# zeux/phyx

Measured on AMD Instinct MI355X. Metric: solver joint-visits/s (contacts/sec) on the 200k-box stack scene; solver iterations/s in extra, higher is better.
Workload: dtype f32

## Files before the change

phyx_amd/csrc/broadphase.hip:

```cpp
#include "handles.h"
#include "device_scan.h"
#include "device_radix.h"
#include "splitter_sort.h"

#include <algorithm>

namespace phx {

static inline int grid_for(int n, int per_block = 256, int cap = 4096) { return std::max(1, std::min(div_up(n, per_block), cap)); }

__device__ __forceinline__ unsigned radix_float(float v)
{
    const int f = __float_as_int(v);
    const unsigned mask = (unsigned)(f >> 31) | 0x80000000u;
    return (unsigned)f ^ mask;
}

__global__ void __launch_bounds__(256) k_extract_aabb(const phx_rigid_body* __restrict__ bodies, int n, float4* __restrict__ aabb)
{
    for (int i = blockIdx.x * blockDim.x + threadIdx.x; i < n; i += gridDim.x * blockDim.x)
        aabb[i] = make_float4(bodies[i].aabb_min.x, bodies[i].aabb_min.y, bodies[i].aabb_max.x, bodies[i].aabb_max.y);
}

template <bool INTEGRATE>
__global__ void __launch_bounds__(256) k_build_keys(const float4* __restrict__ aabb, float4* __restrict__ vel, const float4* __restrict__ mpos, int n,
                                                    unsigned* __restrict__ keys, unsigned* __restrict__ idx,
                                                    unsigned long long* __restrict__ small, int nsmall, unsigned* __restrict__ chunk_count, int nchunks,
                                                    unsigned long long* __restrict__ stamps, float gravity, float dt, unsigned* __restrict__ counters, const float4* __restrict__ accel)
{
    if (INTEGRATE && blockIdx.x == 0 && threadIdx.x < 8) counters[threadIdx.x] = 0u;
    if (blockIdx.x == 0 && threadIdx.x == 0) { stamps[0] = (unsigned long long)wall_clock64(); stamps[1] = 0ull; }
    for (int i = blockIdx.x * blockDim.x + threadIdx.x; i < nsmall; i += gridDim.x * blockDim.x) small[i] = 0ull;
    for (int i = blockIdx.x * blockDim.x + threadIdx.x; i < nchunks; i += gridDim.x * blockDim.x) chunk_count[i] = 0u;
    for (int i = blockIdx.x * blockDim.x + threadIdx.x; i < n; i += gridDim.x * blockDim.x) {
        keys[i] = radix_float(aabb[i].x);
        idx[i] = (unsigned)i;
        if (INTEGRATE) {
            float4 v = vel[i];
            float ax = 0.f, ay = 0.f, aa = 0.f;
            if (accel) { const float4 a = accel[i]; ax = a.x; ay = a.y; aa = a.z; }
            if (mpos[i].x > 0.0f) ay += gravity;
            v.x += ax * dt; v.y += ay * dt;
            v.z += aa * dt;
            vel[i] = v;
        }
    }
}

__global__ void __launch_bounds__(256) k_gather_entries(const float4* __restrict__ aabb, const unsigned* __restrict__ keys, const unsigned* __restrict__ idx, int n,
                                                        float4* __restrict__ entries, unsigned long long* __restrict__ splitters, int stride)
{
    for (int i = blockIdx.x * blockDim.x + threadIdx.x; i < n; i += gridDim.x * blockDim.x) {
        const float4 b = aabb[idx[i]];
        const float minx = b.x, miny = b.y, maxx = b.z, maxy = b.w;
        entries[i] = make_float4(minx, maxx, (miny + maxy) * 0.5f, (maxy - miny) * 0.5f);
        if (i && i % stride == 0) splitters[i / stride - 1] = ((unsigned long long)keys[i] << 32) | idx[i];
    }
}

constexpr unsigned long long PS_EMPTY = 0xFFFFFFFFFFFFFFFFull;
constexpr unsigned long long PS_TOMB = 0xFFFFFFFFFFFFFFFEull;

__device__ __forceinline__ unsigned ps_hash(unsigned long long k)
{
    const unsigned lb = (unsigned)(k >> 32), rb = (unsigned)k;
    return (lb ^ (rb + 0x9e3779b9u + (lb << 6) + (lb >> 2))) * 0x9E3779B1u;
}

__device__ __forceinline__ bool ps_contains(const unsigned long long* __restrict__ table, unsigned mask, unsigned long long k)
{
    unsigned p = ps_hash(k) & mask;
    for (;;) {
        const unsigned long long s = table[p];
        if (s == k) return true;
        if (s == PS_EMPTY) return false;
        p = (p + 1) & mask;
    }
}

__global__ void __launch_bounds__(256) k_ps_insert(unsigned long long* table, unsigned mask, const uint2* __restrict__ pairs, int n, unsigned long long* __restrict__ end_stamp)
{
    for (int i = blockIdx.x * blockDim.x + threadIdx.x; i < n; i += gridDim.x * blockDim.x) {
        const unsigned long long k = ((unsigned long long)pairs[i].x << 32) | pairs[i].y;
        unsigned p = ps_hash(k) & mask;
        for (;;) {
            const unsigned long long s = table[p];
            if (s == PS_EMPTY || s == PS_TOMB) {
                if (atomicCAS(&table[p], s, k) == s) break;
                continue;
            }
            p = (p + 1) & mask;
        }
    }
    if (end_stamp && threadIdx.x == 0) atomicMax(end_stamp, (unsigned long long)wall_clock64());
}

__global__ void __launch_bounds__(256) k_ps_erase(unsigned long long* table, unsigned mask, const uint2* __restrict__ pairs, int n, int* erased)
{
    int mine = 0;
    for (int i = blockIdx.x * blockDim.x + threadIdx.x; i < n; i += gridDim.x * blockDim.x) {
        const unsigned long long k = ((unsigned long long)pairs[i].x << 32) | pairs[i].y;
        unsigned p = ps_hash(k) & mask;
        for (;;) {
            const unsigned long long s = table[p];
            if (s == k) { table[p] = PS_TOMB; ++mine; break; }
            if (s == PS_EMPTY) break;
            p = (p + 1) & mask;
        }
    }
    for (int off = 32; off > 0; off >>= 1) mine += __shfl_down(mine, off);
    if ((threadIdx.x & 63) == 0 && mine) atomicAdd(erased, mine);
}

__global__ void __launch_bounds__(256) k_ps_rehash(const unsigned long long* __restrict__ old_table, unsigned old_cap,
                                                   unsigned long long* table, unsigned mask)
{
    for (unsigned i = blockIdx.x * blockDim.x + threadIdx.x; i < old_cap; i += gridDim.x * blockDim.x) {
        const unsigned long long k = old_table[i];
        if (k == PS_EMPTY || k == PS_TOMB) continue;
        unsigned p = ps_hash(k) & mask;
        for (;;) {
            if (table[p] == PS_EMPTY && atomicCAS(&table[p], PS_EMPTY, k) == PS_EMPTY) break;
            p = (p + 1) & mask;
        }
    }
}

constexpr int STAT_SLOTS = 64;
constexpr int ROW_CACHE = 4;
constexpr int HUB_LEN = 2048;
constexpr int HUB_CHUNK = 512;

struct SweepView {
    const float4* entries;
    const unsigned* idx;
    int n;
    const unsigned long long* table;
    unsigned mask;
    unsigned* row_count;
    unsigned* row_cache;
    int* cache_overflow;
    int4* chunks;
    unsigned* chunk_count;
    int* n_chunks;
    int chunk_cap;
    unsigned long long* counters;
};

struct FilteredSweepView : SweepView {
    const uint4* filters;
};
template <class V> struct SweepFilter { static constexpr bool on = false; };
template <> struct SweepFilter<FilteredSweepView> { static constexpr bool on = true; };
template <class V> __device__ __forceinline__ uint4 sweep_filter_of(const V& v, unsigned body)
{
    if constexpr (SweepFilter<V>::on) return v.filters[body];
    else return make_uint4(0u, 0u, 0u, 0u);
}

constexpr int SWEEP_CAND = 16;
constexpr int SWEEP_LOOK = 8;
constexpr int SWEEP_GROUP = 8;

__device__ __forceinline__ int scan_end(const float4* __restrict__ entries, int n, int i, float maxx)
{
    int lo = i + 1, hi = n;
    while (lo < hi) {
        const int mid = (lo + hi) >> 1;
        if (entries[mid].x > maxx) hi = mid; else lo = mid + 1;
    }
    return lo;
}

#define PHX_SWEEP_WAVE_SYNC() do { __builtin_amdgcn_fence(__ATOMIC_RELEASE, "wavefront"); __builtin_amdgcn_wave_barrier(); __builtin_amdgcn_fence(__ATOMIC_ACQUIRE, "wavefront"); } while (0)

template <bool EMIT, class V>
__global__ void __launch_bounds__(256) k_sweep_rows(V v, const unsigned* __restrict__ row_offset, uint2* __restrict__ out, unsigned total)
{
    __shared__ unsigned cand[SWEEP_CAND][256];
    __shared__ float4 stage[4][2][64];
    unsigned long long tests = 0, overlaps = 0;
    const int lane = threadIdx.x & 63;
    for (int base = blockIdx.x * blockDim.x + (threadIdx.x & ~63); base < v.n; base += gridDim.x * blockDim.x) {
        const int i = base + lane;
        const bool in_range = i < v.n;
        const float4 a = in_range ? v.entries[i] : make_float4(0.f, 0.f, 0.f, 0.f);
        const bool hub = in_range && i + 1 + HUB_LEN < v.n && !(v.entries[i + 1 + HUB_LEN].x > a.y);
        if (!EMIT) {
            int end = 0, nc = 0, first = 0;
            if (hub) {
                end = scan_end(v.entries, v.n, i, a.y);
                const int len = end - i - 1;
                nc = (len + HUB_CHUNK - 1) / HUB_CHUNK;
                first = atomicAdd(v.n_chunks, nc);
                v.row_count[i] = 0;
                tests += (unsigned long long)len;
            }
            for (unsigned long long hubs = __ballot(hub); hubs; hubs &= hubs - 1ull) {
                const int l = __builtin_ctzll(hubs);
                const int hi = __shfl(i, l), hend = __shfl(end, l), hnc = __shfl(nc, l), hfirst = __shfl(first, l);
                for (int k = lane; k < hnc && hfirst + k < v.chunk_cap; k += 64)
                    v.chunks[hfirst + k] = make_int4(hi, hi + 1 + k * HUB_CHUNK, min(hend, hi + 1 + (k + 1) * HUB_CHUNK), hfirst);
            }
        }
        bool scanning = in_range && !hub;
        const unsigned dst = EMIT && scanning ? row_offset[i] : 0u;
        if (EMIT && scanning) {
            const unsigned next = i + 1 < v.n ? row_offset[i + 1] : total;
            if (next - dst <= (unsigned)ROW_CACHE) scanning = false;
        }
        const unsigned ia = scanning ? v.idx[i] : 0u;
        const uint4 fa = scanning ? sweep_filter_of(v, ia) : make_uint4(0u, 0u, 0u, 0u);
        unsigned found = 0;
        int ncand = 0;
        auto flush = [&]() {
            for (int h = 0; h < ncand; h += SWEEP_LOOK) {
                unsigned ib[SWEEP_LOOK];
                unsigned long long first[SWEEP_LOOK];
#pragma unroll
                for (int k = 0; k < SWEEP_LOOK; ++k) ib[k] = h + k < ncand ? v.idx[cand[h + k][threadIdx.x]] : 0u;
                unsigned pass = ~0u;
                if constexpr (SweepFilter<V>::on) {
                    pass = 0u;
#pragma unroll
                    for (int k = 0; k < SWEEP_LOOK; ++k)
                        if (h + k < ncand && collision_filter_pass(fa, sweep_filter_of(v, ib[k]))) pass |= 1u << k;
                }
#pragma unroll
                for (int k = 0; k < SWEEP_LOOK; ++k) first[k] = h + k < ncand && ((pass >> k) & 1u) ? v.table[ps_hash(((unsigned long long)ia << 32) | ib[k]) & v.mask] : 0ull;
#pragma unroll
                for (int k = 0; k < SWEEP_LOOK; ++k) {
                    if (h + k >= ncand) break;
                    if (!((pass >> k) & 1u)) continue;
                    const unsigned long long key = ((unsigned long long)ia << 32) | ib[k];
                    bool present = first[k] == key;
                    if (!present && first[k] != PS_EMPTY) present = ps_contains(v.table, v.mask, key);
                    if (!present) {
                        if (EMIT) out[dst + found] = make_uint2(ia, ib[k]);
                        else if (found < (unsigned)ROW_CACHE) v.row_cache[(size_t)i * ROW_CACHE + found] = ib[k];
                        ++found;
                    }
                }
            }
            ncand = 0;
        };
        int len = 0;
        bool ended = !scanning;
        int ended_w = scanning ? 0 : -1;
        const int c0 = __builtin_amdgcn_readfirstlane(base) + 1;
        float4* my_stage = &stage[threadIdx.x >> 6][0][0];
        float4 nxt = v.entries[min(c0 + lane, v.n - 1)];
        int buf = 0;
        for (int c = c0; c < v.n && __ballot(!ended); c += 64) {
            my_stage[buf * 64 + lane] = nxt;
            if (c + 64 < v.n) nxt = v.entries[min(c + 64 + lane, v.n - 1)];
            PHX_SWEEP_WAVE_SYNC();
            const float4* blockp = my_stage + buf * 64;
            const int rel = i - c;
            for (int g = 0; g < 64 && c + g < v.n && __ballot(!ended); g += SWEEP_GROUP) {
                if (ncand > SWEEP_CAND - SWEEP_GROUP) flush();
                float4 b[SWEEP_GROUP];
#pragma unroll
                for (int k = 0; k < SWEEP_GROUP; ++k) b[k] = blockp[g + k];
#pragma unroll
                for (int k = 0; k < SWEEP_GROUP; ++k) {
                    const int j = c + g + k;
                    const int started = (rel - (g + k)) >> 31;
                    const int in_list = (j - v.n) >> 31;
                    const int beyond = b[k].x > a.y ? -1 : 0;
                    const int live = started & in_list & ~ended_w;
                    ended_w |= live & beyond;
                    const int tested = live & ~beyond;
                    len -= tested;
                    const int ov = (fabsf(b[k].z - a.z) <= a.w + b[k].w ? -1 : 0) & tested;
                    if (__any(ov)) {
                        if (ov) {
                            if (!EMIT) ++overlaps;
                            cand[ncand++][threadIdx.x] = (unsigned)j;
                        }
                    }
                }
                ended = ended_w != 0;
            }
            buf ^= 1;
        }
        if (scanning) {
            flush();
            if (!EMIT) { v.row_count[i] = found; tests += (unsigned long long)len; if (found > (unsigned)ROW_CACHE) *v.cache_overflow = 1; }
        }
    }
    if (!EMIT) {
        for (int off = 32; off > 0; off >>= 1) { tests += __shfl_down(tests, off); overlaps += __shfl_down(overlaps, off); }
        __shared__ unsigned long long part[2][4];
        if ((threadIdx.x & 63) == 0) { part[0][threadIdx.x >> 6] = tests; part[1][threadIdx.x >> 6] = overlaps; }
        __syncthreads();
        if (threadIdx.x < 2) {
            const unsigned long long t = part[threadIdx.x][0] + part[threadIdx.x][1] + part[threadIdx.x][2] + part[threadIdx.x][3];
            if (t) atomicAdd(&v.counters[2 * (blockIdx.x % STAT_SLOTS) + threadIdx.x], t);
        }
    }
}
__device__ __forceinline__ void emit_cached_rows(const SweepView& v, const unsigned* __restrict__ row_offset, uint2* __restrict__ out, unsigned total, int block, int blocks)
{
    for (int i = block * (int)blockDim.x + (int)threadIdx.x; i < v.n; i += blocks * (int)blockDim.x) {
        const unsigned dst = row_offset[i];
        const unsigned count = (i + 1 < v.n ? row_offset[i + 1] : total) - dst;
        if (count == 0 || count > (unsigned)ROW_CACHE) continue;
        if (i + 1 + HUB_LEN < v.n && !(v.entries[i + 1 + HUB_LEN].x > v.entries[i].y)) continue;
        const unsigned ia = v.idx[i];
        for (unsigned k = 0; k < count; ++k) out[dst + k] = make_uint2(ia, v.row_cache[(size_t)i * ROW_CACHE + k]);
    }
}

template <bool EMIT, class V>
__device__ __forceinline__ void sweep_chunks(const V& v, const unsigned* __restrict__ row_offset, uint2* __restrict__ out, int block, int blocks)
{
    __shared__ unsigned wave_cnt[4];
    __shared__ unsigned running;
    const int total = min(*v.n_chunks, v.chunk_cap);
    const int wave = threadIdx.x >> 6, lane = threadIdx.x & 63;
    unsigned long long overlaps_all = 0;
    for (int c = block; c < total; c += blocks) {
        const int4 ch = v.chunks[c];
        const float4 a = v.entries[ch.x];
        const unsigned ia = v.idx[ch.x];
        const uint4 fa = sweep_filter_of(v, ia);
        unsigned long long overlaps = 0;
        if constexpr (!EMIT) {
            unsigned mine = 0;
            for (int j = ch.y + (int)threadIdx.x; j < ch.z; j += 256) {
                const float4 b = v.entries[j];
                if (fabsf(b.z - a.z) <= a.w + b.w) {
                    ++overlaps;
                    const unsigned ib = v.idx[j];
                    if (SweepFilter<V>::on && !collision_filter_pass(fa, sweep_filter_of(v, ib))) continue;
                    if (!ps_contains(v.table, v.mask, ((unsigned long long)ia << 32) | ib)) ++mine;
                }
            }
            for (int off = 32; off > 0; off >>= 1) mine += __shfl_down(mine, off);
            if (lane == 0) wave_cnt[wave] = mine;
            __syncthreads();
            if (threadIdx.x == 0) v.chunk_count[c] = wave_cnt[0] + wave_cnt[1] + wave_cnt[2] + wave_cnt[3];
            overlaps_all += overlaps;
            __syncthreads();
            continue;
        }
        if (threadIdx.x == 0) running = row_offset[ch.x] + v.chunk_count[c];
        __syncthreads();
        for (int j0 = ch.y; j0 < ch.z; j0 += 256) {
            const int j = j0 + threadIdx.x;
            bool hit = false;
            unsigned ib = 0;
            if (j < ch.z) {
                const float4 b = v.entries[j];
                if (fabsf(b.z - a.z) <= a.w + b.w) {
                    ib = v.idx[j];
                    ++overlaps;
                    hit = (!SweepFilter<V>::on || collision_filter_pass(fa, sweep_filter_of(v, ib))) && !ps_contains(v.table, v.mask, ((unsigned long long)ia << 32) | ib);
                }
            }
            const unsigned long long bal = __ballot(hit);
            if (lane == 0) wave_cnt[wave] = (unsigned)__popcll(bal);
            __syncthreads();
            unsigned before = 0;
            for (int w = 0; w < wave; ++w) before += wave_cnt[w];
            const unsigned base = running;
            if (EMIT && hit) out[base + before + (unsigned)__popcll(bal & ((1ull << lane) - 1ull))] = make_uint2(ia, ib);
            __syncthreads();
            if (threadIdx.x == 0) running = base + wave_cnt[0] + wave_cnt[1] + wave_cnt[2] + wave_cnt[3];
            __syncthreads();
        }
        __syncthreads();
    }
    if (!EMIT) {
        for (int off = 32; off > 0; off >>= 1) overlaps_all += __shfl_down(overlaps_all, off);
        if (lane == 0 && overlaps_all) atomicAdd(&v.counters[2 * ((block * 4 + wave) % STAT_SLOTS) + 1], overlaps_all);
    }
}

template <class V>
__global__ void __launch_bounds__(256) k_sweep_chunks_count(V v) { sweep_chunks<false>(v, nullptr, nullptr, (int)blockIdx.x, (int)gridDim.x); }

template <class V>
__global__ void __launch_bounds__(256) k_emit_pairs(V v, const unsigned* __restrict__ row_offset, uint2* __restrict__ out, unsigned total, int row_blocks)
{
    if ((int)blockIdx.x < row_blocks) emit_cached_rows(v, row_offset, out, total, (int)blockIdx.x, row_blocks);
    else sweep_chunks<true>(v, row_offset, out, (int)blockIdx.x - row_blocks, (int)gridDim.x - row_blocks);
}

__global__ void __launch_bounds__(1024) k_chunk_bases(SweepView v, unsigned* __restrict__ scanned)
{
    __shared__ unsigned lds[16];
    __shared__ unsigned tot;
    const int total = min(*v.n_chunks, v.chunk_cap);
    unsigned carry = 0;
    for (int tile = 0; tile < total; tile += 1024) {
        const int c = tile + (int)threadIdx.x;
        const unsigned mine = c < total ? v.chunk_count[c] : 0u;
        const unsigned ex = block_exclusive_scan_1024(mine, lds, threadIdx.x == 0 ? &tot : nullptr);
        if (c < total) scanned[c] = carry + ex;
        __syncthreads();
        carry += tot;
        __syncthreads();
    }
    __threadfence_block();
    __syncthreads();
    for (int c = threadIdx.x; c < total; c += 1024) {
        const int4 ch = v.chunks[c];
        const unsigned count = v.chunk_count[c];
        const bool last = (c + 1 == total) || v.chunks[c + 1].x != ch.x;
        if (last) v.row_count[ch.x] = scanned[c] + count - scanned[ch.w];
    }
    __syncthreads();
    for (int c = threadIdx.x; c < total; c += 1024) v.chunk_count[c] = scanned[c] - scanned[v.chunks[c].w];
}

__global__ void __launch_bounds__(256) k_entries_to_aos(const float4* __restrict__ entries, const unsigned* __restrict__ keys,
                                                        const unsigned* __restrict__ idx, int n,
                                                        phx_broadphase_entry* __restrict__ out_entries, phx_sort_entry* __restrict__ out_sorted)
{
    for (int i = blockIdx.x * blockDim.x + threadIdx.x; i < n; i += gridDim.x * blockDim.x) {
        const float4 e = entries[i];
        out_entries[i].minx = e.x; out_entries[i].maxx = e.y; out_entries[i].centery = e.z; out_entries[i].extenty = e.w;
        out_entries[i].index = idx[i];
        out_sorted[i].value = keys[i]; out_sorted[i].index = idx[i];
    }
}


DeviceBroadphase::~DeviceBroadphase()
{
    if (hipSetDevice(device_) != hipSuccess) return;
    if (stream_) (void)hipStreamSynchronize(stream_);
    if (stream_) (void)hipStreamDestroy(stream_);
}

int DeviceBroadphase::init()
{
    PHX_TRY(use_device(device_));
    PHX_HIP(hipStreamCreateWithFlags(&stream_, hipStreamNonBlocking));
    PHX_TRY(small_.reserve(16 + 2 * STAT_SLOTS));
    PHX_TRY(erase_count_.reserve(1));
    PHX_HIP(hipMemsetAsync(erase_count_.p, 0, sizeof(int), stream_));
    return clear();
}

int DeviceBroadphase::exclusive_scan(unsigned* data, int count, unsigned* total_out)
{
    return device_exclusive_scan(data, count, total_out, scan_tiles_, stream_);
}

int DeviceBroadphase::resize_table(unsigned want_cap)
{
    unsigned cap = 1024;
    while (cap < want_cap) cap <<= 1;
    DevBuf<unsigned long long> fresh;
    PHX_TRY(fresh.reserve(cap));
    PHX_HIP(hipMemsetAsync(fresh.p, 0xFF, (size_t)cap * sizeof(unsigned long long), stream_));
    if (table_.p && table_cap_) {
        hipLaunchKernelGGL(k_ps_rehash, dim3(grid_for((int)table_cap_)), dim3(256), 0, stream_, table_.p, table_cap_, fresh.p, cap - 1);
        PHX_HIP(hipGetLastError());
    }
    PHX_HIP(hipStreamSynchronize(stream_));
    table_ = std::move(fresh);
    table_cap_ = cap;
    tombstones_ = 0;
    return PHX_OK;
}

int DeviceBroadphase::clear()
{
    PHX_TRY(use_device(device_));
    table_.release();
    table_cap_ = 0;
    set_size_ = 0;
    tombstones_ = 0;
    if (erase_unchecked_) { erase_unchecked_ = 0; PHX_HIP(hipMemsetAsync(erase_count_.p, 0, sizeof(int), stream_)); }
    return resize_table(1024);
}

int DeviceBroadphase::update_device(const phx_rigid_body* d_bodies, int n)
{
    PHX_TRY(use_device(device_));
    PHX_REQUIRE(n >= 0 && (n == 0 || d_bodies), "bad body array");
    PHX_TRY(st_aabb_.reserve(std::max(n, 1)));
    if (n) hipLaunchKernelGGL(k_extract_aabb, dim3(grid_for(n)), dim3(256), 0, stream_, d_bodies, n, st_aabb_.p);
    PHX_HIP(hipGetLastError());
    return update_resident(st_aabb_.p, n);
}

int DeviceBroadphase::update_resident(const float4* d_bodies, int n, const StepPrologue* prologue, const std::function<int()>* while_waiting, const MailCarrier* carrier,
                                      const uint4* filters)
{
    PHX_TRY(use_device(device_));
    PHX_REQUIRE(n >= 0 && (n == 0 || d_bodies), "bad body array");
    n_ = n;
    last_new_ = 0;
    stats_ = phx_broadphase_stats{};
    for (int k = 0; k < 2; ++k) { PHX_TRY(keys_[k].reserve(std::max(n, 1))); PHX_TRY(idx_[k].reserve(std::max(n, 1))); }
    PHX_TRY(hist_.reserve(radix_hist_words(n)));
    int chunk_cap = std::max<int>((int)chunks_.cap, div_up(std::max(n, 1), HUB_CHUNK) * 8 + 64);
    PHX_TRY(chunks_.reserve(chunk_cap));
    PHX_TRY(chunk_count_.reserve(chunk_cap));
    PHX_TRY(entries_.reserve(std::max(n, 1)));
    PHX_TRY(row_count_.reserve(std::max(n, 1) + 1));
    PHX_TRY(row_cache_.reserve((size_t)std::max(n, 1) * ROW_CACHE));
    if ((unsigned long long)(set_size_ + tombstones_) * 2 > table_cap_) PHX_TRY(resize_table((unsigned)std::max<long long>(4 * set_size_, 1024)));

    PHX_TRY(stamps_.reserve(2));
    if (n == 0) {
        if (prologue) PHX_HIP(hipMemsetAsync(prologue->counters, 0, 8 * sizeof(unsigned), stream_));
        PHX_HIP(hipMemsetAsync(stamps_.p, 0, 2 * sizeof(unsigned long long), stream_));
        PHX_HIP(hipStreamSynchronize(stream_));
        stats_.candidate_tests = 0; stats_.overlapping_pairs = 0; stats_.new_pairs = 0; last_new_ = 0;
        stats_.set_size = (int)set_size_; have_update_ = true; ms_pending_ = true;
        return PHX_OK;
    }

    const int buckets = ss_buckets(n);
    const bool appended = splitters_n_ == n && splitters_from_ > 0 && splitters_from_ < n;
    const int deal = appended ? ss_buckets(splitters_from_) : buckets;
    PHX_TRY(splitters_.reserve(SS_MAX_BUCKETS)); PHX_TRY(ss_stats_.reserve(2));
    static const bool no_split = getenv("PHX_NO_SPLIT_SORT") != nullptr;
    const bool split = !no_split && buckets <= SS_MAX_BUCKETS && (buckets == 1 || (splitters_n_ == n && !split_unbalanced_ && (!appended || n <= 2 * splitters_from_)));
    int src = 0;
    if (split) {
        if (!ss_count_.p) { PHX_TRY(ss_count_.reserve(2 * SS_MAX_BUCKETS)); PHX_HIP(hipMemsetAsync(ss_count_.p, 0, ss_count_.cap * sizeof(unsigned), stream_)); }
        PHX_TRY(ss_base_.reserve(SS_MAX_BUCKETS + 1)); PHX_TRY(bucket_of_.reserve(n)); PHX_TRY(bucketed_.reserve(n));
        SplitSortView sv{};
        sv.aabb = d_bodies; sv.n = n; sv.buckets = deal; sv.stride = ss_stride(n); sv.splitters = splitters_.p; sv.keys = keys_[0].p; sv.bucket_of = bucket_of_.p;
        sv.count = ss_count_.p; sv.cursor = ss_count_.p + SS_MAX_BUCKETS; sv.base = ss_base_.p; sv.bucketed = bucketed_.p;
        sv.keys_out = keys_[1].p; sv.idx_out = idx_[1].p; sv.entries = entries_.p; sv.next_splitters = splitters_.p; sv.max_bucket = ss_stats_.p;
        const int items = ss_tile_items(deal);
        const dim3 tiles(div_up(n, SS_TILE_T * items));
#define PHX_KEYS_BUCKETS(INTEGRATE, ITEMS, ...) hipLaunchKernelGGL((k_keys_buckets<INTEGRATE, ITEMS>), tiles, dim3(SS_TILE_T), 0, stream_, sv, __VA_ARGS__)
        if (prologue) {
            if (items == SS_ITEMS_LARGE) PHX_KEYS_BUCKETS(true, SS_ITEMS_LARGE, prologue->vel, prologue->mpos, small_.p, 16 + 2 * STAT_SLOTS, chunk_count_.p, chunk_cap, stamps_.p, prologue->gravity, prologue->dt, prologue->counters, prologue->accel);
            else PHX_KEYS_BUCKETS(true, SS_ITEMS_SMALL, prologue->vel, prologue->mpos, small_.p, 16 + 2 * STAT_SLOTS, chunk_count_.p, chunk_cap, stamps_.p, prologue->gravity, prologue->dt, prologue->counters, prologue->accel);
        } else {
            if (items == SS_ITEMS_LARGE) PHX_KEYS_BUCKETS(false, SS_ITEMS_LARGE, (float4*)nullptr, (const float4*)nullptr, small_.p, 16 + 2 * STAT_SLOTS, chunk_count_.p, chunk_cap, stamps_.p, 0.f, 0.f, (unsigned*)nullptr, (const float4*)nullptr);
            else PHX_KEYS_BUCKETS(false, SS_ITEMS_SMALL, (float4*)nullptr, (const float4*)nullptr, small_.p, 16 + 2 * STAT_SLOTS, chunk_count_.p, chunk_cap, stamps_.p, 0.f, 0.f, (unsigned*)nullptr, (const float4*)nullptr);
        }
#undef PHX_KEYS_BUCKETS
        if (items == SS_ITEMS_LARGE) hipLaunchKernelGGL((k_bucket_scatter<SS_ITEMS_LARGE>), tiles, dim3(SS_TILE_T), 0, stream_, sv);
        else hipLaunchKernelGGL((k_bucket_scatter<SS_ITEMS_SMALL>), tiles, dim3(SS_TILE_T), 0, stream_, sv);
        if (ss_last_max_ <= (unsigned)SS_LDS_SMALL_LIMIT) hipLaunchKernelGGL((k_bucket_sort<SS_LDS_SMALL>), dim3(deal), dim3(SS_SORT_T), 0, stream_, sv);
        else hipLaunchKernelGGL((k_bucket_sort<SS_LDS_RECORDS>), dim3(deal), dim3(SS_SORT_T), 0, stream_, sv);
        src = 1;
    } else {
        if (prologue) hipLaunchKernelGGL((k_build_keys<true>), dim3(grid_for(n)), dim3(256), 0, stream_, d_bodies, prologue->vel, prologue->mpos, n, keys_[0].p, idx_[0].p, small_.p, 16 + 2 * STAT_SLOTS,
                                         chunk_count_.p, chunk_cap, stamps_.p, prologue->gravity, prologue->dt, prologue->counters, prologue->accel);
        else hipLaunchKernelGGL((k_build_keys<false>), dim3(grid_for(n)), dim3(256), 0, stream_, d_bodies, (float4*)nullptr, (const float4*)nullptr, n, keys_[0].p, idx_[0].p, small_.p, 16 + 2 * STAT_SLOTS,
                                chunk_count_.p, chunk_cap, stamps_.p, 0.f, 0.f, (unsigned*)nullptr, (const float4*)nullptr);
        PHX_TRY(device_radix_sort_pairs(keys_[0].p, idx_[0].p, keys_[1].p, idx_[1].p, n, 32, hist_.p, scan_tiles_, stream_, &src));
        hipLaunchKernelGGL(k_gather_entries, dim3(grid_for(n)), dim3(256), 0, stream_, d_bodies, (const unsigned*)keys_[src].p, (const unsigned*)idx_[src].p, n, entries_.p, splitters_.p, ss_stride(n));
        PHX_HIP(hipMemsetAsync(ss_stats_.p, 0, sizeof(unsigned), stream_));
        split_unbalanced_ = false;
    }
    sorted_ = src;
    splitters_n_ = n; splitters_from_ = n;
    split_sorted_ = split;

    SweepView v{};
    v.entries = entries_.p; v.idx = idx_[src].p; v.n = n; v.table = table_.p; v.mask = table_cap_ - 1;
    v.row_count = row_count_.p; v.row_cache = row_cache_.p; v.cache_overflow = reinterpret_cast<int*>(small_.p + 4);
    v.n_chunks = reinterpret_cast<int*>(small_.p + 2);
    v.counters = small_.p + 16;
    unsigned long long host_small[16 + 2 * STAT_SLOTS] = {0};
    int chunk_grid = 1;
    for (int attempt = 0;; ++attempt) {
        v.chunks = chunks_.p; v.chunk_count = chunk_count_.p; v.chunk_cap = chunk_cap;
        chunk_grid = std::min(chunk_cap, 2048);
        if (filters) {
            const FilteredSweepView fv{v, filters};
            hipLaunchKernelGGL((k_sweep_rows<false, FilteredSweepView>), dim3(grid_for(n)), dim3(256), 0, stream_, fv, (const unsigned*)nullptr, (uint2*)nullptr, 0u);
            hipLaunchKernelGGL((k_sweep_chunks_count<FilteredSweepView>), dim3(chunk_grid), dim3(256), 0, stream_, fv);
        } else {
            hipLaunchKernelGGL((k_sweep_rows<false, SweepView>), dim3(grid_for(n)), dim3(256), 0, stream_, v, (const unsigned*)nullptr, (uint2*)nullptr, 0u);
            hipLaunchKernelGGL((k_sweep_chunks_count<SweepView>), dim3(chunk_grid), dim3(256), 0, stream_, v);
        }
        PHX_TRY(chunk_scan_.reserve(chunk_cap + 1));
        hipLaunchKernelGGL(k_chunk_bases, dim3(1), dim3(1024), 0, stream_, v, chunk_scan_.p);
        PHX_TRY(exclusive_scan(row_count_.p, n, reinterpret_cast<unsigned*>(small_.p + 3)));
        PHX_HIP(hipGetLastError());
        int erased = 0;
        PHX_TRY(queue_erase_check(&erased));
        PHX_TRY(rb_.add(host_small, small_.p, sizeof host_small, stream_));
        unsigned max_bucket = 0;
        if (split) PHX_TRY(rb_.add(&max_bucket, ss_stats_.p, sizeof max_bucket, stream_));
        PHX_TRY(rb_.wait(stream_, stamps_.p + 1, attempt == 0 ? while_waiting : nullptr, attempt == 0 ? carrier : nullptr));
        PHX_TRY(settle_erase_check(erased));
        ss_last_max_ = split ? max_bucket : 0u;
        if (split && max_bucket > (unsigned)(4 * ss_stride(n))) split_unbalanced_ = true;
        const int needed = (int)(host_small[2] & 0xFFFFFFFFull);
        if (needed <= chunk_cap) break;
        if (attempt) { set_error("broadphase: hub chunk list overflow twice (%d chunks)", needed); return PHX_ERR_CAPACITY; }
        chunk_cap = needed + 64;
        PHX_TRY(chunks_.reserve(chunk_cap));
        PHX_TRY(chunk_count_.reserve(chunk_cap));
        PHX_HIP(hipMemsetAsync(small_.p, 0, (16 + 2 * STAT_SLOTS) * sizeof(unsigned long long), stream_));
        PHX_HIP(hipMemsetAsync(chunk_count_.p, 0, (size_t)chunk_cap * sizeof(unsigned), stream_));
    }
    const unsigned total = (unsigned)host_small[3];
    stats_.candidate_tests = 0; stats_.overlapping_pairs = 0;
    for (int k = 0; k < STAT_SLOTS; ++k) { stats_.candidate_tests += (long long)host_small[16 + 2 * k]; stats_.overlapping_pairs += (long long)host_small[17 + 2 * k]; }
    stats_.new_pairs = (int)total;
    last_new_ = (int)total;
    if (total) {
        PHX_TRY(new_pairs_.reserve(total));
        if ((unsigned long long)(set_size_ + tombstones_ + (long long)total) * 2 > table_cap_)
            PHX_TRY(resize_table((unsigned)std::min<long long>(4ll * (set_size_ + (long long)total), 1ll << 30)));
        v.table = table_.p; v.mask = table_cap_ - 1;
        {
            const int row_blocks = grid_for(n), chunk_blocks = (host_small[2] & 0xFFFFFFFFull) ? std::min((int)(host_small[2] & 0xFFFFFFFFull), chunk_grid) : 0;
            if (filters) hipLaunchKernelGGL((k_emit_pairs<FilteredSweepView>), dim3(row_blocks + chunk_blocks), dim3(256), 0, stream_, FilteredSweepView{v, filters}, (const unsigned*)row_count_.p, new_pairs_.p, total, row_blocks);
            else hipLaunchKernelGGL((k_emit_pairs<SweepView>), dim3(row_blocks + chunk_blocks), dim3(256), 0, stream_, v, (const unsigned*)row_count_.p, new_pairs_.p, total, row_blocks);
        }
        if (host_small[4] & 0xFFFFFFFFull) {
            if (filters) hipLaunchKernelGGL((k_sweep_rows<true, FilteredSweepView>), dim3(grid_for(n)), dim3(256), 0, stream_, FilteredSweepView{v, filters}, (const unsigned*)row_count_.p, new_pairs_.p, total);
            else hipLaunchKernelGGL((k_sweep_rows<true, SweepView>), dim3(grid_for(n)), dim3(256), 0, stream_, v, (const unsigned*)row_count_.p, new_pairs_.p, total);
        }
        hipLaunchKernelGGL(k_ps_insert, dim3(grid_for((int)total)), dim3(256), 0, stream_, table_.p, table_cap_ - 1, (const uint2*)new_pairs_.p, (int)total, stamps_.p + 1);
        PHX_HIP(hipGetLastError());
        set_size_ += total;
    }
    stats_.set_size = (int)set_size_;
    have_update_ = true;
    ms_pending_ = true;
    return PHX_OK;
}

int DeviceBroadphase::update_host(const phx_rigid_body* bodies, int n, uint32_t* new_pairs, int cap, int* count)
{
    PHX_TRY(use_device(device_));
    PHX_REQUIRE(n >= 0 && (n == 0 || bodies), "bad body array");
    PHX_TRY(st_bodies_.reserve(std::max(n, 1)));
    if (n) PHX_HIP(hipMemcpyAsync(st_bodies_.p, bodies, (size_t)n * sizeof(phx_rigid_body), hipMemcpyHostToDevice, stream_));
    PHX_TRY(update_device(st_bodies_.p, n));
    PHX_HIP(hipStreamSynchronize(stream_));
    return get_new_pairs(new_pairs, cap, count);
}

int DeviceBroadphase::get_new_pairs(uint32_t* out, int cap, int* count)
{
    if (!have_update_) { set_error("no broadphase update has run yet"); return PHX_ERR_STATE; }
    if (count) *count = last_new_;
    if (!out) return PHX_OK;
    if (cap < last_new_) { set_error("new-pair buffer too small: need %d", last_new_); return PHX_ERR_CAPACITY; }
    PHX_TRY(use_device(device_));
    PHX_HIP(hipStreamSynchronize(stream_));
    if (last_new_) PHX_HIP(hipMemcpy(out, new_pairs_.p, (size_t)last_new_ * sizeof(uint2), hipMemcpyDeviceToHost));
    return PHX_OK;
}

int DeviceBroadphase::get_sorted(phx_sort_entry* sorted, phx_broadphase_entry* entries, int cap)
{
    if (!have_update_) { set_error("no broadphase update has run yet"); return PHX_ERR_STATE; }
    if (cap < n_) { set_error("sorted buffers too small: need %d", n_); return PHX_ERR_CAPACITY; }
    PHX_TRY(use_device(device_));
    if (!n_) return PHX_OK;
    DevBuf<phx_broadphase_entry> de;
    DevBuf<phx_sort_entry> ds;
    PHX_TRY(de.reserve(n_));
    PHX_TRY(ds.reserve(n_));
    hipLaunchKernelGGL(k_entries_to_aos, dim3(grid_for(n_)), dim3(256), 0, stream_, (const float4*)entries_.p, (const unsigned*)keys_[sorted_].p,
                       (const unsigned*)idx_[sorted_].p, n_, de.p, ds.p);
    PHX_HIP(hipGetLastError());
    if (entries) PHX_HIP(hipMemcpyAsync(entries, de.p, (size_t)n_ * sizeof(phx_broadphase_entry), hipMemcpyDeviceToHost, stream_));
    if (sorted) PHX_HIP(hipMemcpyAsync(sorted, ds.p, (size_t)n_ * sizeof(phx_sort_entry), hipMemcpyDeviceToHost, stream_));
    PHX_HIP(hipStreamSynchronize(stream_));
    de.release();
    ds.release();
    return PHX_OK;
}

int DeviceBroadphase::erase_pairs_device(const uint2* d_pairs, int count)
{
    PHX_TRY(use_device(device_));
    PHX_REQUIRE(count >= 0 && (count == 0 || d_pairs), "bad pair list");
    if (!count) return PHX_OK;
    hipLaunchKernelGGL(k_ps_erase, dim3(grid_for(count)), dim3(256), 0, stream_, table_.p, table_cap_ - 1, d_pairs, count, erase_count_.p);
    PHX_HIP(hipGetLastError());
    set_size_ -= count;
    tombstones_ += count;
    erase_unchecked_ += count;
    return PHX_OK;
}

int DeviceBroadphase::reset_pairs(const uint2* pairs, int count)
{
    PHX_TRY(use_device(device_));
    PHX_REQUIRE(count >= 0 && (count == 0 || pairs), "bad pair list");
    if (count) {
        PHX_TRY(scratch_pairs_.reserve((size_t)count));
        PHX_HIP(hipMemcpyAsync(scratch_pairs_.p, pairs, (size_t)count * sizeof(uint2), hipMemcpyHostToDevice, stream_));
    }
    PHX_TRY(reset_pairs_device(scratch_pairs_.p, count));
    PHX_HIP(hipStreamSynchronize(stream_));
    return PHX_OK;
}

int DeviceBroadphase::reset_pairs_device(const uint2* d_pairs, int count)
{
    PHX_TRY(use_device(device_));
    PHX_REQUIRE(count >= 0 && (count == 0 || d_pairs), "bad pair list");
    PHX_TRY(clear());
    have_update_ = false;
    if (!count) return PHX_OK;
    PHX_TRY(resize_table(4u * (unsigned)count + 1024u));
    hipLaunchKernelGGL(k_ps_insert, dim3(grid_for(count)), dim3(256), 0, stream_, table_.p, table_cap_ - 1, d_pairs, count, (unsigned long long*)nullptr);
    PHX_HIP(hipGetLastError());
    set_size_ = count;
    stats_.set_size = count;
    return PHX_OK;
}

int DeviceBroadphase::queue_erase_check(int* erased)
{
    *erased = 0;
    if (!erase_unchecked_) return PHX_OK;
    return rb_.add(erased, erase_count_.p, sizeof(int), stream_);
}

int DeviceBroadphase::settle_erase_check(int erased)
{
    if (!erase_unchecked_) return PHX_OK;
    const long long missing = erase_unchecked_ - erased;
    set_size_ += missing;
    tombstones_ = std::max<long long>(0, tombstones_ - missing);
    erase_unchecked_ = 0;
    PHX_HIP(hipMemsetAsync(erase_count_.p, 0, sizeof(int), stream_));
    return PHX_OK;
}

int DeviceBroadphase::erase_pairs(const uint32_t* pairs, int count)
{
    PHX_TRY(use_device(device_));
    PHX_REQUIRE(count >= 0 && (count == 0 || pairs), "bad pair list");
    if (!count) return PHX_OK;
    PHX_TRY(scratch_pairs_.reserve(count));
    PHX_HIP(hipMemcpyAsync(scratch_pairs_.p, pairs, (size_t)count * sizeof(uint2), hipMemcpyHostToDevice, stream_));
    return erase_pairs_device(scratch_pairs_.p, count);
}

int DeviceBroadphase::get_stats(phx_broadphase_stats* out)
{
    PHX_REQUIRE(out, "null out");
    if (!have_update_) { set_error("no broadphase update has run yet"); return PHX_ERR_STATE; }
    PHX_TRY(use_device(device_));
    if (ms_pending_) {
        unsigned long long stamps[2] = {0, 0};
        PHX_TRY(rb_.add(stamps, stamps_.p, sizeof stamps, stream_));
        PHX_TRY(rb_.wait(stream_));
        stats_.device_ms = stamps[1] > stamps[0] ? (double)(stamps[1] - stamps[0]) * 1e-5 : 0.0;
        ms_pending_ = false;
    }
    if (erase_unchecked_) {
        int erased = 0;
        PHX_TRY(queue_erase_check(&erased));
        PHX_TRY(rb_.wait(stream_));
        PHX_TRY(settle_erase_check(erased));
    }
    *out = stats_;
    out->set_size = (int)set_size_;
    return PHX_OK;
}

}


extern "C" {

int phx_broadphase_create(phx_broadphase** out, int device)
{
    PHX_REQUIRE(out, "null out");
    *out = nullptr;
    PHX_TRY(phx::use_device(device));
    phx_broadphase* b = new (std::nothrow) phx_broadphase(device);
    PHX_REQUIRE(b, "out of host memory");
    int st = b->impl.init();
    if (st != PHX_OK) { delete b; return st; }
    *out = b;
    return PHX_OK;
}

void phx_broadphase_destroy(phx_broadphase* b) { delete b; }

int phx_broadphase_clear(phx_broadphase* b) { PHX_REQUIRE(b, "null handle"); return b->impl.clear(); }

int phx_broadphase_update(phx_broadphase* b, const phx_rigid_body* bodies, int32_t n, uint32_t* new_pairs, int32_t cap, int32_t* count)
{
    PHX_REQUIRE(b, "null handle");
    return b->impl.update_host(bodies, n, new_pairs, cap, count);
}

int phx_broadphase_update_device(phx_broadphase* b, const void* d_bodies, int32_t n)
{
    PHX_REQUIRE(b, "null handle");
    return b->impl.update_device(static_cast<const phx_rigid_body*>(d_bodies), n);
}

int phx_broadphase_get_sorted(phx_broadphase* b, phx_sort_entry* sorted, phx_broadphase_entry* entries, int32_t cap)
{
    PHX_REQUIRE(b, "null handle");
    return b->impl.get_sorted(sorted, entries, cap);
}

int phx_broadphase_get_new_pairs(phx_broadphase* b, uint32_t* new_pairs, int32_t cap, int32_t* count)
{
    PHX_REQUIRE(b, "null handle");
    return b->impl.get_new_pairs(new_pairs, cap, count);
}

int phx_broadphase_erase_pairs(phx_broadphase* b, const uint32_t* pairs, int32_t count)
{
    PHX_REQUIRE(b, "null handle");
    return b->impl.erase_pairs(pairs, count);
}

int phx_broadphase_get_stats(phx_broadphase* b, phx_broadphase_stats* out)
{
    PHX_REQUIRE(b, "null handle");
    return b->impl.get_stats(out);
}

}
```

Before: 116.8 billion.

## Fuse pair-set insertion into broadphase emit kernels and drop separate insert pass

New pairs are now inserted into the persistent pair hash table right where they are written out (emit_cached_rows, sweep_chunks, and the emit variant of k_sweep_rows), and the separate k_ps_insert launch after emission is removed. The end timestamp moves into whichever emit kernel runs last, and only a subset of blocks issue the atomicMax. This saves one kernel launch and a re-read of the new-pairs buffer. The risk is that emit kernels probing the table with ps_contains now race with concurrent inserts into the same table, and the insert loop was changed to reuse the CAS return value.

Result: no change. 116.9 billion (median of 3 runs) (+0.1%).

```diff
diff --git a/phyx_amd/csrc/broadphase.hip b/phyx_amd/csrc/broadphase.hip
--- a/phyx_amd/csrc/broadphase.hip
+++ b/phyx_amd/csrc/broadphase.hip
@@ -78,21 +78,31 @@
     }
 }
 
-__global__ void __launch_bounds__(256) k_ps_insert(unsigned long long* table, unsigned mask, const uint2* __restrict__ pairs, int n, unsigned long long* __restrict__ end_stamp)
-{
-    for (int i = blockIdx.x * blockDim.x + threadIdx.x; i < n; i += gridDim.x * blockDim.x) {
-        const unsigned long long k = ((unsigned long long)pairs[i].x << 32) | pairs[i].y;
-        unsigned p = ps_hash(k) & mask;
-        for (;;) {
-            const unsigned long long s = table[p];
-            if (s == PS_EMPTY || s == PS_TOMB) {
-                if (atomicCAS(&table[p], s, k) == s) break;
-                continue;
-            }
-            p = (p + 1) & mask;
-        }
-    }
-    if (end_stamp && threadIdx.x == 0) atomicMax(end_stamp, (unsigned long long)wall_clock64());
+__device__ __forceinline__ void ps_insert_key(unsigned long long* table, unsigned mask, unsigned long long k)
+{
+    unsigned p = ps_hash(k) & mask;
+    unsigned long long s = table[p];
+    for (;;) {
+        if (s == PS_EMPTY || s == PS_TOMB) {
+            const unsigned long long was = atomicCAS(&table[p], s, k);
+            if (was == s) return;
+            s = was;
+            continue;
+        }
+        p = (p + 1) & mask;
+        s = table[p];
+    }
+}
+
+__device__ __forceinline__ void stamp_end(unsigned long long* __restrict__ end_stamp)
+{
+    if (end_stamp && threadIdx.x == 0 && ((blockIdx.x & 63u) == 0u || blockIdx.x + 1 == gridDim.x)) atomicMax(end_stamp, (unsigned long long)wall_clock64());
+}
+
+__global__ void __launch_bounds__(256) k_ps_insert(unsigned long long* table, unsigned mask, const uint2* __restrict__ pairs, int n)
+{
+    for (int i = blockIdx.x * blockDim.x + threadIdx.x; i < n; i += gridDim.x * blockDim.x)
+        ps_insert_key(table, mask, ((unsigned long long)pairs[i].x << 32) | pairs[i].y);
 }
 
 __global__ void __launch_bounds__(256) k_ps_erase(unsigned long long* table, unsigned mask, const uint2* __restrict__ pairs, int n, int* erased)
@@ -135,7 +145,7 @@
     const float4* entries;
     const unsigned* idx;
     int n;
-    const unsigned long long* table;
+    unsigned long long* table;
     unsigned mask;
     unsigned* row_count;
     unsigned* row_cache;
@@ -175,7 +185,7 @@
 #define PHX_SWEEP_WAVE_SYNC() do { __builtin_amdgcn_fence(__ATOMIC_RELEASE, "wavefront"); __builtin_amdgcn_wave_barrier(); __builtin_amdgcn_fence(__ATOMIC_ACQUIRE, "wavefront"); } while (0)
 
 template <bool EMIT, class V>
-__global__ void __launch_bounds__(256) k_sweep_rows(V v, const unsigned* __restrict__ row_offset, uint2* __restrict__ out, unsigned total)
+__global__ void __launch_bounds__(256) k_sweep_rows(V v, const unsigned* __restrict__ row_offset, uint2* __restrict__ out, unsigned total, unsigned long long* __restrict__ end_stamp)
 {
     __shared__ unsigned cand[SWEEP_CAND][256];
     __shared__ float4 stage[4][2][64];
@@ -236,7 +246,7 @@
                     bool present = first[k] == key;
                     if (!present && first[k] != PS_EMPTY) present = ps_contains(v.table, v.mask, key);
                     if (!present) {
-                        if (EMIT) out[dst + found] = make_uint2(ia, ib[k]);
+                        if (EMIT) { out[dst + found] = make_uint2(ia, ib[k]); ps_insert_key(v.table, v.mask, key); }
                         else if (found < (unsigned)ROW_CACHE) v.row_cache[(size_t)i * ROW_CACHE + found] = ib[k];
                         ++found;
                     }
@@ -299,6 +309,7 @@
             if (t) atomicAdd(&v.counters[2 * (blockIdx.x % STAT_SLOTS) + threadIdx.x], t);
         }
     }
+    if (EMIT) stamp_end(end_stamp);
 }
 __device__ __forceinline__ void emit_cached_rows(const SweepView& v, const unsigned* __restrict__ row_offset, uint2* __restrict__ out, unsigned total, int block, int blocks)
 {
@@ -308,7 +319,11 @@
         if (count == 0 || count > (unsigned)ROW_CACHE) continue;
         if (i + 1 + HUB_LEN < v.n && !(v.entries[i + 1 + HUB_LEN].x > v.entries[i].y)) continue;
         const unsigned ia = v.idx[i];
-        for (unsigned k = 0; k < count; ++k) out[dst + k] = make_uint2(ia, v.row_cache[(size_t)i * ROW_CACHE + k]);
+        for (unsigned k = 0; k < count; ++k) {
+            const unsigned ib = v.row_cache[(size_t)i * ROW_CACHE + k];
+            out[dst + k] = make_uint2(ia, ib);
+            ps_insert_key(v.table, v.mask, ((unsigned long long)ia << 32) | ib);
+        }
     }
 }
 
@@ -365,7 +380,10 @@
             unsigned before = 0;
             for (int w = 0; w < wave; ++w) before += wave_cnt[w];
             const unsigned base = running;
-            if (EMIT && hit) out[base + before + (unsigned)__popcll(bal & ((1ull << lane) - 1ull))] = make_uint2(ia, ib);
+            if (EMIT && hit) {
+                out[base + before + (unsigned)__popcll(bal & ((1ull << lane) - 1ull))] = make_uint2(ia, ib);
+                ps_insert_key(v.table, v.mask, ((unsigned long long)ia << 32) | ib);
+            }
             __syncthreads();
             if (threadIdx.x == 0) running = base + wave_cnt[0] + wave_cnt[1] + wave_cnt[2] + wave_cnt[3];
             __syncthreads();
@@ -382,10 +400,12 @@
 __global__ void __launch_bounds__(256) k_sweep_chunks_count(V v) { sweep_chunks<false>(v, nullptr, nullptr, (int)blockIdx.x, (int)gridDim.x); }
 
 template <class V>
-__global__ void __launch_bounds__(256) k_emit_pairs(V v, const unsigned* __restrict__ row_offset, uint2* __restrict__ out, unsigned total, int row_blocks)
+__global__ void __launch_bounds__(256) k_emit_pairs(V v, const unsigned* __restrict__ row_offset, uint2* __restrict__ out, unsigned total, int row_blocks,
+                                                    unsigned long long* __restrict__ end_stamp)
 {
     if ((int)blockIdx.x < row_blocks) emit_cached_rows(v, row_offset, out, total, (int)blockIdx.x, row_blocks);
     else sweep_chunks<true>(v, row_offset, out, (int)blockIdx.x - row_blocks, (int)gridDim.x - row_blocks);
+    stamp_end(end_stamp);
 }
 
 __global__ void __launch_bounds__(1024) k_chunk_bases(SweepView v, unsigned* __restrict__ scanned)
@@ -573,10 +593,10 @@
         chunk_grid = std::min(chunk_cap, 2048);
         if (filters) {
             const FilteredSweepView fv{v, filters};
-            hipLaunchKernelGGL((k_sweep_rows<false, FilteredSweepView>), dim3(grid_for(n)), dim3(256), 0, stream_, fv, (const unsigned*)nullptr, (uint2*)nullptr, 0u);
+            hipLaunchKernelGGL((k_sweep_rows<false, FilteredSweepView>), dim3(grid_for(n)), dim3(256), 0, stream_, fv, (const unsigned*)nullptr, (uint2*)nullptr, 0u, (unsigned long long*)nullptr);
             hipLaunchKernelGGL((k_sweep_chunks_count<FilteredSweepView>), dim3(chunk_grid), dim3(256), 0, stream_, fv);
         } else {
-            hipLaunchKernelGGL((k_sweep_rows<false, SweepView>), dim3(grid_for(n)), dim3(256), 0, stream_, v, (const unsigned*)nullptr, (uint2*)nullptr, 0u);
+            hipLaunchKernelGGL((k_sweep_rows<false, SweepView>), dim3(grid_for(n)), dim3(256), 0, stream_, v, (const unsigned*)nullptr, (uint2*)nullptr, 0u, (unsigned long long*)nullptr);
             hipLaunchKernelGGL((k_sweep_chunks_count<SweepView>), dim3(chunk_grid), dim3(256), 0, stream_, v);
         }
         PHX_TRY(chunk_scan_.reserve(chunk_cap + 1));
@@ -611,16 +631,17 @@
         if ((unsigned long long)(set_size_ + tombstones_ + (long long)total) * 2 > table_cap_)
             PHX_TRY(resize_table((unsigned)std::min<long long>(4ll * (set_size_ + (long long)total), 1ll << 30)));
         v.table = table_.p; v.mask = table_cap_ - 1;
+        const bool rescan = (host_small[4] & 0xFFFFFFFFull) != 0;
+        unsigned long long* const emit_stamp = rescan ? nullptr : stamps_.p + 1;
         {
             const int row_blocks = grid_for(n), chunk_blocks = (host_small[2] & 0xFFFFFFFFull) ? std::min((int)(host_small[2] & 0xFFFFFFFFull), chunk_grid) : 0;
-            if (filters) hipLaunchKernelGGL((k_emit_pairs<FilteredSweepView>), dim3(row_blocks + chunk_blocks), dim3(256), 0, stream_, FilteredSweepView{v, filters}, (const unsigned*)row_count_.p, new_pairs_.p, total, row_blocks);
-            else hipLaunchKernelGGL((k_emit_pairs<SweepView>), dim3(row_blocks + chunk_blocks), dim3(256), 0, stream_, v, (const unsigned*)row_count_.p, new_pairs_.p, total, row_blocks);
-        }
-        if (host_small[4] & 0xFFFFFFFFull) {
-            if (filters) hipLaunchKernelGGL((k_sweep_rows<true, FilteredSweepView>), dim3(grid_for(n)), dim3(256), 0, stream_, FilteredSweepView{v, filters}, (const unsigned*)row_count_.p, new_pairs_.p, total);
-            else hipLaunchKernelGGL((k_sweep_rows<true, SweepView>), dim3(grid_for(n)), dim3(256), 0, stream_, v, (const unsigned*)row_count_.p, new_pairs_.p, total);
-        }
-        hipLaunchKernelGGL(k_ps_insert, dim3(grid_for((int)total)), dim3(256), 0, stream_, table_.p, table_cap_ - 1, (const uint2*)new_pairs_.p, (int)total, stamps_.p + 1);
+            if (filters) hipLaunchKernelGGL((k_emit_pairs<FilteredSweepView>), dim3(row_blocks + chunk_blocks), dim3(256), 0, stream_, FilteredSweepView{v, filters}, (const unsigned*)row_count_.p, new_pairs_.p, total, row_blocks, emit_stamp);
+            else hipLaunchKernelGGL((k_emit_pairs<SweepView>), dim3(row_blocks + chunk_blocks), dim3(256), 0, stream_, v, (const unsigned*)row_count_.p, new_pairs_.p, total, row_blocks, emit_stamp);
+        }
+        if (rescan) {
+            if (filters) hipLaunchKernelGGL((k_sweep_rows<true, FilteredSweepView>), dim3(grid_for(n)), dim3(256), 0, stream_, FilteredSweepView{v, filters}, (const unsigned*)row_count_.p, new_pairs_.p, total, stamps_.p + 1);
+            else hipLaunchKernelGGL((k_sweep_rows<true, SweepView>), dim3(grid_for(n)), dim3(256), 0, stream_, v, (const unsigned*)row_count_.p, new_pairs_.p, total, stamps_.p + 1);
+        }
         PHX_HIP(hipGetLastError());
         set_size_ += total;
     }
@@ -708,7 +729,7 @@
     have_update_ = false;
     if (!count) return PHX_OK;
     PHX_TRY(resize_table(4u * (unsigned)count + 1024u));
-    hipLaunchKernelGGL(k_ps_insert, dim3(grid_for(count)), dim3(256), 0, stream_, table_.p, table_cap_ - 1, d_pairs, count, (unsigned long long*)nullptr);
+    hipLaunchKernelGGL(k_ps_insert, dim3(grid_for(count)), dim3(256), 0, stream_, table_.p, table_cap_ - 1, d_pairs, count);
     PHX_HIP(hipGetLastError());
     set_size_ = count;
     stats_.set_size = count;
```
